# manuelinfosec/corrosion

Measured on AMD Instinct MI355X. Metric: merged column-changes/sec (node) at 1/2/4/8 GPUs + % of HBM BW roofline, higher is better.
Workload: dtype int64; 1 GPU; config 2: 64M column-changes, 1 table x 4 INTEGER cols, 1000 actors, uniform pk in [1,2^22], cl=1, one apply into an empty state per step; changes=67108864, cells=16469597, parallelism=1 GPU

## Files before the change

corrosion_amd/csrc/engine.hip:

```cpp
#include <hip/hip_runtime.h>

#include <algorithm>
#include <chrono>
#include <cstdlib>
#include <cstring>
#include <mutex>
#include <numeric>

#include "internal.h"
#include "merge_kernels.h"

namespace corro {

static thread_local std::string g_last_error;

void set_error(const std::string &msg) { g_last_error = msg; }

int fail(int code, const std::string &msg) {
    g_last_error = msg;
    return code;
}

int DevBuf::ensure(size_t want) {
    if (want <= bytes && p) return CORRO_OK;
// ... 411 lines not shown
        return fail(CORRO_E_NO_DEVICE, std::string("libcorro_hip is built for gfx950, device is ") + prop.gcnArchName);
    CORRO_HIP_TRY(hipStreamCreateWithFlags(&ctx->stream, hipStreamNonBlocking));
    CORRO_HIP_TRY(hipHostMalloc((void **)&ctx->h_misc, MISC_WORDS * sizeof(uint64_t), hipHostMallocDefault));
    CORRO_HIP_TRY(hipHostGetDevicePointer((void **)&ctx->h_misc_dev, ctx->h_misc, 0));
    for (auto &e : ctx->ev) CORRO_HIP_TRY(hipEventCreate(&e));
    const size_t lds_max = 160 * 1024;
    for (const void *f : {(const void *)k_hist<8>, (const void *)k_hist<16>, (const void *)k_hist<32>,
                          (const void *)k_hist<16, true>, (const void *)k_hist<16, false, true>})
        CORRO_HIP_TRY(hipFuncSetAttribute(f, hipFuncAttributeMaxDynamicSharedMemorySize, (int)lds_max));
    for (const void *f : {(const void *)k_scatter<true, true>, (const void *)k_scatter<true, false>,
                          (const void *)k_scatter<true, false, 8>,
                          (const void *)k_scatter<false, true>, (const void *)k_scatter<false, false>})
        CORRO_HIP_TRY(hipFuncSetAttribute(f, hipFuncAttributeMaxDynamicSharedMemorySize, (int)lds_max));
    return CORRO_OK;
}

}

static int store_alloc(corro_ctx *ctx, uint64_t capacity_hint) {
    const uint32_t B = ctx->B;
    const uint64_t rows = std::max<uint64_t>(1024, capacity_hint / 16);
    uint32_t lg = 4;
    while (((uint64_t)B << lg) < 2 * rows && lg < 20 && ((uint64_t)B << (lg + 1)) <= (1ULL << 31)) lg++;
    ctx->log2S = lg;
    TRY(ctx->d_ent.ensure(((size_t)B << lg) * sizeof(RowEnt)));
    TRY(ctx->d_used.ensure(B * 4ULL));
    TRY(ctx->d_gen.ensure(B * 4ULL));
    TRY(ctx->d_heap_top.ensure(8));
    ctx->heap_cap = std::min<uint64_t>(1ULL << 31, std::max<uint64_t>(1ULL << 16, capacity_hint / 2));
    TRY(ctx->d_heap.ensure(ctx->heap_cap * sizeof(Rec)));
    return CORRO_OK;
}

static int store_clear(corro_ctx *ctx) {
    hipStream_t s = ctx->stream;
    const size_t n16 = ((size_t)ctx->B << ctx->log2S) * (sizeof(RowEnt) / 16);
    static const uint32_t grid_max = std::getenv("CORRO_CLEAR_GRID") ? (uint32_t)std::atoi(std::getenv("CORRO_CLEAR_GRID")) : CLEAR_GRID;
    static const bool nt = !std::getenv("CORRO_CLEAR_NT") || std::atoi(std::getenv("CORRO_CLEAR_NT")) != 0;
    const uint32_t grid = (uint32_t)std::min<size_t>(std::max(grid_max, 1u), (n16 + CLEAR_T - 1) / CLEAR_T);
    hipLaunchKernelGGL(nt ? k_store_clear<true> : k_store_clear<false>, dim3(std::max(grid, 1u)), dim3(CLEAR_T), 0, s,
                       row_store(ctx), ctx->B, ctx->d_touch_n.as<unsigned long long>());
    CORRO_HIP_TRY(hipGetLastError());
    ctx->touch_bound = 0;
    ctx->state_total = 0;
    ctx->state_rows = 0;
    ctx->arena_top = 0;
    ctx->vc_last_bytes = 0;
    ctx->state_epoch++;
    ctx->poisoned = false;
    return CORRO_OK;
}

namespace corro {
RowStore row_store(corro_ctx *ctx) {
    RowStore rs{};
    rs.ent = ctx->d_ent.as<RowEnt>();
    rs.used = ctx->d_used.as<uint32_t>();
    rs.gen = ctx->d_gen.as<uint32_t>();
    rs.heap = ctx->d_heap.as<Rec>();
    rs.heap_ts = ctx->track_ts ? ctx->d_heap_ts.as<uint64_t>() : nullptr;
    rs.heap_top = ctx->d_heap_top.as<unsigned long long>();
    rs.heap_cap = ctx->heap_cap;
    rs.log2S = ctx->log2S;
    rs.fill = (uint32_t)((7ULL << ctx->log2S) >> 3);
    rs.stride = ctx->d_stride.as<uint16_t>();
    return rs;
}

static constexpr uint64_t ARENA_MAX = 1ULL << 40;
int arena_reserve(corro_ctx *ctx, uint64_t add) {
    const uint64_t need = ctx->arena_top + add;
    if (need > ARENA_MAX) return fail(CORRO_E_RANGE, "value arena would exceed 2^40 bytes");
    if (need <= ctx->d_arena.bytes && ctx->d_arena.p) return CORRO_OK;
    DevBuf nb;
    TRY(nb.ensure(std::max<uint64_t>(need + (need >> 1), 1ULL << 20)));
    if (ctx->arena_top)
        CORRO_HIP_TRY(hipMemcpyAsync(nb.p, ctx->d_arena.p, ctx->arena_top, hipMemcpyDeviceToDevice, ctx->stream));
    CORRO_HIP_TRY(hipStreamSynchronize(ctx->stream));
    ctx->d_arena.release();
    ctx->d_arena = nb;
    nb.p = nullptr;
    return CORRO_OK;
}

int grow_regions(corro_ctx *ctx, uint32_t new_log2S) {
    if (new_log2S <= ctx->log2S) return CORRO_OK;
    ctx->metrics.region_growths++;
    if (new_log2S > 26 || ((uint64_t)ctx->B << new_log2S) > (1ULL << 31))
        return fail(CORRO_E_NOMEM, "row store regions would exceed 2^31 entries");
    hipStream_t s = ctx->stream;
    DevBuf nb;
    TRY(nb.ensure(((size_t)ctx->B << new_log2S) * sizeof(RowEnt)));
    CORRO_HIP_TRY(hipMemsetAsync(nb.p, 0, ((size_t)ctx->B << new_log2S) * sizeof(RowEnt), s));
    const uint32_t old_log2S = ctx->log2S;
    DevBuf old = ctx->d_ent;
    ctx->d_ent = nb;
    nb.p = nullptr;
// ... 1090 lines not shown
```

corrosion_amd/csrc/internal.h:

```cpp
#pragma once
#include <hip/hip_runtime.h>

#include <array>
#include <cstdint>
#include <cstdlib>
#include <map>
#include <string>
#include <unordered_map>
#include <vector>

#include "corro_hip.h"

namespace corro {

inline bool fault_armed(const char *name) {
    const char *e = std::getenv("CORRO_FAULT");
    if (!e || !*e) return false;
    const std::string s = std::string(",") + e + ",";
    return s.find(std::string(",") + name + ",") != std::string::npos;
}

void set_error(const std::string &msg);
int fail(int code, const std::string &msg);

// ... 108 lines not shown
        if (o == 0xFFFFFFFFu) return o;
        if (t.lo[h] == lo && t.hi[h] == hi) return o;
        h = (h + 1) & t.mask;
    }
}

int prims_warm(corro_ctx *ctx);
int agent_dev_reserve(corro_ctx *ctx, uint64_t ncs);

}

struct corro_ctx {
    int device = 0;
    hipStream_t stream = nullptr;
    std::vector<corro::Table> tables;
    std::vector<corro::PkTable> pk;
    std::map<std::string, uint32_t> table_index;

    std::vector<std::array<uint8_t, 16>> sites;
    std::map<std::array<uint8_t, 16>, uint32_t> site_ordinal;
    corro::DevBuf d_site_rank;
    corro::DevBuf d_dbv;
    corro::DevBuf d_dbv_batch;
    size_t dbv_cap = 0;

    uint32_t log2B = 0;
    uint32_t B = 0;
    corro::DevBuf d_ent;
    corro::DevBuf d_used, d_gen;
    corro::DevBuf d_heap, d_heap_ts;
    corro::DevBuf d_heap_top;
    corro::DevBuf d_stride;
    uint32_t log2S = 0;
    uint64_t heap_cap = 0;
    uint32_t max_stride = 1;
    uint64_t state_total = 0;
    uint64_t state_rows = 0;
    corro_metrics metrics{};
    std::vector<uint64_t> committed;
    bool track_ts = false;
    bool track_touched = false;
    corro::DevBuf d_touch, d_touch_n, d_touch_stamp, d_touch_tmp;
    uint64_t touch_cap = 0;
    uint64_t touch_bound = 0;
    uint32_t touch_epoch = 0;
    uint64_t touch_stamp_n = 0;
    bool poisoned = false;
    uint64_t dbv_writes = 0;
    const uint32_t *pm_ap = nullptr, *pm_src = nullptr;
    const uint64_t *pm_ts = nullptr;
    uint64_t pm_n = 0;
    bool pm_slack = false;
    const void *slot_rec = nullptr;
    const uint64_t *slot_cnt = nullptr;
    uint32_t slot_cap = 0, slot_nsrc = 0;
    uint32_t *slot_over = nullptr;
    bool apply_wrote = false;
    uint64_t heap_limit = 0;
    bool state_wide = false;
    corro::DevBuf d_defer, d_relist;
    corro::DevBuf d_dense, d_dense_ts, d_dense_view;
    corro::DevBuf d_arena;
    uint64_t arena_top = 0;
    uint64_t vc_min_bytes = 0;
    uint64_t vc_last_bytes = 0;
    uint64_t dense_epoch = ~0ULL;
// ... 81 lines not shown
```

corrosion_amd/csrc/merge_kernels.h:

```cpp
#pragma once
#include "internal.h"
#include "rowhash.h"
#include "rowstore.h"

namespace corro {

#ifndef CORRO_DIAG
#define CORRO_DIAG 0
#endif
constexpr int HIST_THREADS = 512;
constexpr uint64_t CV_PACKED_LIMIT = 1ULL << 15;
constexpr uint32_t TILES_MAX = 256;
constexpr int MERGE_THREADS = 512;
#ifndef CORRO_FAST_T
#define CORRO_FAST_T 512
#endif
constexpr int FAST_T = CORRO_FAST_T;
constexpr int CAP_FAST = 3072;
constexpr int FAST_R = CAP_FAST / FAST_T;
static_assert(FAST_R * FAST_T == CAP_FAST, "FAST_T must divide CAP_FAST");
constexpr int FAST_WAVES_EU = 2 * (FAST_T / 64) / 4;
constexpr int FAST_SLOTS = 4096;
#ifndef IMPACT_LISTS
#define IMPACT_LISTS 0
// ... 1116 lines not shown
        if (i < n && row[k] == i) {
            s_heap[i] = 0x80000000u | off;
            off += strd[k];
        }
    }
    rows = wave_sum_u32(rows);
    if ((tid & 63) == 0 && rows) atomicAdd(&s_ctl[0], rows);
}

__device__ inline void fast_rows_alloc(const MergeArgs &a, uint32_t b, uint32_t used0, uint32_t *s_ctl,
                                       unsigned long long *s_hbase) {
    bool ok = used0 + s_ctl[0] <= a.rs.fill;
    unsigned long long h = 0;
    if (ok && s_ctl[1]) {
#if CORRO_DIAG & 8
        h = (unsigned long long)b * 640u;
#else
        h = rs_heap_alloc(a.rs, s_ctl[1]);
#endif
        ok = h != ~0ULL;
    }
    if (!ok) {
        push_defer(a, b, used0 + s_ctl[0] <= a.rs.fill ? DEFER_HEAP : DEFER_REGION);
        s_ctl[2] = 1;
    } else {
        a.rs.used[b] = used0 + s_ctl[0];
        *s_hbase = h;
    }
}

template <int R>
__device__ inline bool fast_rows(const MergeArgs &a, uint32_t b, uint32_t used0, uint32_t n, const uint32_t (&row)[R],
                                 uint32_t (&ent)[R], const uint64_t *s_pk, const uint32_t *s_tc, uint32_t *s_heap,
                                 uint64_t *s_bits, uint32_t *s_ctl, unsigned long long *s_hbase, bool counted) {
    const uint32_t tid = threadIdx.x;
    const uint32_t S = 1u << a.rs.log2S;
    uint32_t *s_bm = s_heap + CAP_FAST;
    const bool lds_claim = S <= 32 * RS_BM_WORDS;
    if (lds_claim)
        for (uint32_t w = tid; w < (S + 31) / 32; w += FAST_T) s_bm[w] = 0;
    uint32_t e0[R], hw[R];
#pragma unroll
    for (int k = 0; k < R; k++) {
        const uint32_t i = k * FAST_T + tid;
        ent[k] = ROW_NONE;
        e0[k] = 0;
        hw[k] = 0;
        if (i >= n || row[k] != i) continue;
        const uint64_t pk = s_pk[i];
        const uint32_t t = s_tc[i] >> 16;
        if (counted) {
            hw[k] = s_heap[i];
            s_bits[i] = 0;
            e0[k] = region_slot(pk, t, a.rs.log2S);
            ent[k] = ROW_NONE - 1;
            continue;
        }
        const uint32_t e = used0 ? rs_probe(a.rs, b, pk, t, e0[k]) : ROW_NONE;
        if (!used0) e0[k] = region_slot(pk, t, a.rs.log2S);
        if (e != ROW_NONE) {
            hw[k] = a.rs.ent[e].heap;
            s_bits[i] = a.rs.ent[e].bits[0];
            ent[k] = e;
        } else {
            hw[k] = (uint32_t)a.rs.stride[t];
            s_bits[i] = 0;
            ent[k] = ROW_NONE - 1;
// ... 14 lines not shown
                const uint32_t st = hw[k];
                hw[k] = 0x80000000u | off;
                off += st;
            }
        rows = wave_sum_u32(rows);
        if ((tid & 63) == 0 && rows) atomicAdd(&s_ctl[0], rows);
    }
    __syncthreads();
    if (!counted) {
#pragma unroll
        for (int k = 0; k < R; k++)
            if (ent[k] != ROW_NONE) s_heap[k * FAST_T + tid] = hw[k];
        if (tid == 0) fast_rows_alloc(a, b, used0, s_ctl, s_hbase);
        __syncthreads();
    }
    if (s_ctl[2]) return false;
#pragma unroll
    for (int k = 0; k < R; k++) {
        const uint32_t i = k * FAST_T + tid;
        if (ent[k] != ROW_NONE - 1) continue;
#if CORRO_DIAG & 2
        ent[k] = ROW_NONE;
        continue;
#endif
        const uint32_t t = s_tc[i] >> 16, hb = row_heap(hw[k], *s_hbase);
        if (!lds_claim) {
            ent[k] = rs_claim(a.rs, b, e0[k], s_pk[i], t, hb);
            continue;
        }
        uint32_t sl = e0[k];
        while (true) {
            const uint32_t bit = 1u << (sl & 31);
            if (!(atomicOr(&s_bm[sl >> 5], bit) & bit) &&
                (sl == e0[k] || !used0 || a.rs.ent[((size_t)b << a.rs.log2S) + sl].tag == 0))
                break;
            sl = (sl + 1) & (S - 1);
        }
        const uint32_t e = (b << a.rs.log2S) | sl;
        RowEnt &re = a.rs.ent[e];
        re.pk = s_pk[i];
        re.tag = t + 1;
        re.heap = hb;
        re.bits[1] = 0;
        ent[k] = e;
    }
    return true;
}

__device__ inline int prior_cmp_int(const MergeArgs &a, const Rec &pr, uint64_t cvb, uint64_t v0b, uint32_t rank) {
    const uint64_t pcv = (uint64_t)pr.cv ^ 0x8000000000000000ULL, pv = pr.v0 ^ 0x8000000000000000ULL;
    if (cvb != pcv) return cvb > pcv ? 1 : -1;
    if (v0b != pv) return v0b > pv ? 1 : -1;
    const uint32_t pr_rank = site_rank_of(a, pr.site);
    return rank != pr_rank ? (rank > pr_rank ? 1 : -1) : 0;
}

template <bool WIDE>
__device__ inline void fast_body(const MergeArgs &a, uint32_t b, const BucketView &v, bool packed = false) {
    __shared__ uint64_t s_pk[CAP_FAST];
    __shared__ uint64_t s_k[CAP_FAST];
    __shared__ uint32_t s_tc[CAP_FAST];
    __shared__ uint32_t s_own[FAST_SLOTS];
    __shared__ uint32_t s_ctl[4];
    __shared__ unsigned long long s_hbase, s_live;
    const uint32_t tid = threadIdx.x;
    const uint32_t n = v.nn;
    uint64_t cv[FAST_R], v0[FAST_R], v1[FAST_R], rp[FAST_R], dbv[FAST_R];
    uint32_t meta[FAST_R], cell[FAST_R], seq[FAST_R], site[FAST_R], row[FAST_R];
    bool alive[FAST_R];
    uint4 q[FAST_R][4];
#if CORRO_DIAG & 64
    unsigned long long diag_t = wall_clock64();
#define DIAG_MARK(k) do { if (tid == 0) { const unsigned long long t_ = wall_clock64(); atomicAdd(&a.misc[MISC_DIAG + (k)], t_ - diag_t); diag_t = t_; } } while (0)
#else
#define DIAG_MARK(k) do { } while (0)
// ... 110 lines not shown
#pragma unroll
        for (int k = 0; k < FAST_R; k++) {
            w[k] = 0;
            if (!alive[k]) continue;
            const uint32_t ty = WIDE ? vtype(meta[k]) : (uint32_t)CORRO_INTEGER;
            const bool tb = ty == CORRO_TEXT || ty == CORRO_BLOB;
            switch (which) {
            case 0: w[k] = cv[k]; break;
            case 1: w[k] = 5u - ty; break;
            case 2: w[k] = vkey0(ty, v0[k]); break;
            case 3: w[k] = tb ? v1[k] : 0; break;
            case 4: w[k] = tb ? vlen(meta[k]) : 0; break;
            default: w[k] = rp[k]; break;
            }
            atomicMax(reinterpret_cast<unsigned long long *>(&s_k[cell[k]]), (unsigned long long)w[k]);
        }
        __syncthreads();
        if (st == 0 && !used0 && tid == 0) fast_rows_alloc(a, b, used0, s_ctl, &s_hbase);
#pragma unroll
        for (int k = 0; k < FAST_R; k++)
            if (alive[k]) alive[k] = s_k[cell[k]] == w[k];
        __syncthreads();
        if (st + 1 < nstages) {
#pragma unroll
            for (int k = 0; k < FAST_R; k++) {
                const uint32_t i = k * FAST_T + tid;
                if (i < n && cell[k] == i) s_k[i] = 0;
            }
            __syncthreads();
        }
    }
    DIAG_MARK(2);
    uint32_t ent[FAST_R];
    if (!fast_rows<FAST_R>(a, b, used0, n, row, ent, s_pk, s_tc, s_own, s_k, s_ctl, &s_hbase, used0 == 0)) return;
    DIAG_MARK(3);
    uint32_t hb[FAST_R];
    uint32_t nlive = 0;
#pragma unroll
    for (int k = 0; k < FAST_R; k++) {
        hb[k] = 0;
        if (!alive[k]) continue;
        const uint32_t i = k * FAST_T + tid;
        const uint32_t c = s_tc[i] & 0xFFFFu;
        hb[k] = row_heap(s_own[row[k]], s_hbase) + c;
        if ((s_k[row[k]] >> c) & 1ULL) {
            const Rec pr = load_rec(a.rs.heap + hb[k]);
            int cmp;
            if (WIDE) {
                Rec x = load_rec(v.fresh + i);
                cmp = (int64_t)(cv[k] ^ 0x8000000000000000ULL) != pr.cv
                          ? ((int64_t)(cv[k] ^ 0x8000000000000000ULL) > pr.cv ? 1 : -1)
                          : value_cmp(x, pr, a.arena);
                if (cmp == 0) {
                    const uint32_t rk = (uint32_t)(rp[k] >> 32), prk = site_rank_of(a, pr.site);
                    cmp = rk != prk ? (rk > prk ? 1 : -1) : 0;
                }
            } else {
                cmp = prior_cmp_int(a, pr, cv[k], v0[k] ^ 0x8000000000000000ULL, (uint32_t)(rp[k] >> 32));
            }
            if (cmp <= 0) alive[k] = false;
        } else {
            atomicOr(reinterpret_cast<unsigned long long *>(&s_k[row[k]]), 1ULL << c);
            nlive++;
        }
    }
#pragma unroll
    for (int k = 0; k < FAST_R; k++) {
// ... 84 lines not shown
        alive[k] = i < n;
        cell[k] = 0;
        const Rec r = rec_from_wave_quads(q[k]);
        pk[k] = r.pk;
        tc[k] = r.tcid;
        s_pk[i] = r.pk;
        s_tc[i] = r.tcid;
        cv[k] = (uint64_t)r.cv ^ 0x8000000000000000ULL;
        v0[k] = r.v0;
        v1[k] = r.v1;
        meta[k] = r.meta;
        pos[k] = r.pos;
        site[k] = r.site;
        dbv[k] = (uint64_t)r.dbv;
        seq[k] = r.seq;
    }
#pragma unroll
    for (int k = 0; k < FAST_R; k++) rank[k] = a.site_rank[site[k] < a.nsites ? site[k] : 0u];
#pragma unroll
    for (int k = 0; k < FAST_R; k++) rank[k] = site[k] < a.nsites ? rank[k] : 0u;
    __syncthreads();
#pragma unroll
    for (int k = 0; k < FAST_R; k++) {
        const uint32_t i = k * FAST_T + tid;
        row[k] = 0;
        if (!alive[k]) continue;
        row[k] = row_claim(reinterpret_cast<uint32_t *>(s_v0), s_pk, s_tc, i, pk[k], tc[k] >> 16);
    }
    __syncthreads();
#pragma unroll
    for (int k = 0; k < FAST_R; k++)
        if (alive[k]) cell[k] = cell_claim(s_own, k * FAST_T + tid, row[k], tc[k]);
    __syncthreads();
    if (!fast_rows<FAST_R>(a, b, used0, n, row, ent, s_pk, s_tc, s_own, s_v0, s_ctl, &s_hbase, false)) return;
#pragma unroll
    for (int k = 0; k < FAST_R; k++) {
        hb[k] = 0;
        if (!alive[k]) continue;
        const uint32_t c = tc[k] & 0xFFFFu;
        hb[k] = row_heap(s_own[row[k]], s_hbase) + c;
        if ((s_v0[row[k]] >> c) & 1ULL) {
            const Rec pr = load_rec(a.rs.heap + hb[k]);
            const int64_t bcv = (int64_t)(cv[k] ^ 0x8000000000000000ULL);
            int cmp = bcv != pr.cv ? (bcv > pr.cv ? 1 : -1) : value_cmp_f(meta[k], v0[k], v1[k], pr.meta, pr.v0, pr.v1, a.arena);
            if (cmp == 0) {
                const uint32_t prk = site_rank_of(a, pr.site);
                cmp = rank[k] != prk ? (rank[k] > prk ? 1 : -1) : 0;
            }
            if (cmp > 0) flags |= 1u << (2 * k);
        } else {
            flags |= 3u << (2 * k);
        }
    }
    __syncthreads();
    for (uint32_t i = tid; i < FAST_SLOTS; i += FAST_T) s_own[i] = 0;
    __syncthreads();
#pragma unroll
    for (int k = 0; k < FAST_R; k++) {
        const uint32_t i = k * FAST_T + tid;
        if (!alive[k]) continue;
        s_pk[i] = cv[k];
        s_tc[i] = rank[k];
        s_v0[i] = v0[k];
        s_pos[i] = pos[k];
        s_v1[i] = v1[k];
        s_meta[i] = meta[k];
        atomicAdd(&s_own[cell[k]], 1u);
// ... 150 lines not shown
        alive[k] = i < n;
        cell[k] = 0;
        const Rec r = rec_from_wave_quads(q[k]);
        pk[k] = r.pk;
        tc[k] = r.tcid;
        s_a[i] = r.pk;
        s_b[i] = r.tcid;
        cv[k] = (uint64_t)r.cv ^ 0x8000000000000000ULL;
        v0[k] = r.v0 ^ 0x8000000000000000ULL;
        pos[k] = r.pos;
        site[k] = r.site;
        dbv[k] = (uint64_t)r.dbv;
        seq[k] = r.seq;
    }
#pragma unroll
    for (int k = 0; k < FAST_R; k++) rank[k] = a.site_rank[site[k] < a.nsites ? site[k] : 0u];
#pragma unroll
    for (int k = 0; k < FAST_R; k++) rank[k] = site[k] < a.nsites ? rank[k] : 0u;
    __syncthreads();
    DIAG_MARK2(0);
#pragma unroll
    for (int k = 0; k < FAST_R; k++) {
        const uint32_t i = k * FAST_T + tid;
        row[k] = 0;
        if (!alive[k]) continue;
        row[k] = row_claim(reinterpret_cast<uint32_t *>(s_c), s_a, s_b, i, pk[k], tc[k] >> 16);
    }
    __syncthreads();
#pragma unroll
    for (int k = 0; k < FAST_R; k++)
        if (alive[k]) cell[k] = cell_claim(s_own, k * FAST_T + tid, row[k], tc[k]);
    __syncthreads();
    DIAG_MARK2(1);
    if (!fast_rows<FAST_R>(a, b, used0, n, row, ent, s_a, s_b, s_own, s_c, s_ctl, &s_hbase, false)) return;
    DIAG_MARK2(2);
#pragma unroll
    for (int k = 0; k < FAST_R; k++) {
        hb[k] = 0;
        if (!alive[k]) continue;
        const uint32_t c = tc[k] & 0xFFFFu;
        hb[k] = row_heap(s_own[row[k]], s_hbase) + c;
        if ((s_c[row[k]] >> c) & 1ULL) {
            const Rec pr = load_rec(a.rs.heap + hb[k]);
            if (prior_cmp_int(a, pr, cv[k], v0[k], rank[k]) > 0) flags |= 1u << (2 * k);
        } else {
            flags |= 3u << (2 * k);
        }
    }
    __syncthreads();
    DIAG_MARK2(3);
    for (uint32_t i = tid; i < FAST_SLOTS; i += FAST_T) s_own[i] = 0;
    __syncthreads();
#pragma unroll
    for (int k = 0; k < FAST_R; k++)
        if (alive[k]) atomicAdd(&s_own[cell[k]], 1u);
    __syncthreads();
    {
        const uint32_t i0 = tid * FAST_R;
        uint32_t c[FAST_R], loc = 0;
#pragma unroll
        for (int k = 0; k < FAST_R; k++) {
            c[k] = i0 + k < n ? s_own[i0 + k] : 0u;
            loc += c[k];
        }
        const uint32_t lane = tid & 63, w = tid >> 6;
        uint32_t inc = loc;
#pragma unroll
// ... 167 lines not shown
        strd[k] = used0 ? 0u : (uint32_t)a.rs.stride[alive[k] ? tc[k] >> 16 : 0u];
        k2[k] |= a.site_rank[site[k] < a.nsites ? site[k] : 0u];
    }
#pragma unroll
    for (int k = 0; k < FAST_R; k++)
        if (site[k] >= a.nsites) k2[k] &= 0xFFFF0000u;
    __syncthreads();
    DIAG_MARK2(0);
#pragma unroll
    for (int k = 0; k < FAST_R; k++) {
        const uint32_t i = k * FAST_T + tid;
        row[k] = 0;
        if (!alive[k]) continue;
        row[k] = row_claim(reinterpret_cast<uint32_t *>(s_c), s_a, s_b, i, s_a[i], tc[k] >> 16);
    }
    __syncthreads();
#pragma unroll
    for (int k = 0; k < FAST_R; k++)
        if (alive[k]) cell[k] = cell_claim(s_own, k * FAST_T + tid, row[k], tc[k]);
    __syncthreads();
    DIAG_MARK2(1);
    unsigned long long hraw = 0;
    if (!used0) {
        fast_rows_count<FAST_R>(n, row, strd, s_own, s_ctl);
        __syncthreads();
#pragma unroll
        for (int k = 0; k < FAST_R; k++) {
            hb[k] = alive[k] ? (s_own[row[k]] & 0x7FFFFFFFu) + (tc[k] & 0xFFFFu) : 0u;
            ent[k] = ROW_NONE;
            if (alive[k]) flags |= 3u << (2 * k);
        }
        if (tid == 0 && s_ctl[1] && s_ctl[0] <= a.rs.fill) hraw = atomicAdd(a.rs.heap_top, (unsigned long long)s_ctl[1]);
    } else {
        if (!fast_rows<FAST_R>(a, b, used0, n, row, ent, s_a, s_b, s_own, s_c, s_ctl, &s_hbase, false)) return;
#pragma unroll
        for (int k = 0; k < FAST_R; k++) {
            hb[k] = 0;
            if (!alive[k]) continue;
            const uint32_t c = tc[k] & 0xFFFFu;
            hb[k] = row_heap(s_own[row[k]], s_hbase) + c;
            if ((s_c[row[k]] >> c) & 1ULL) {
                const Rec pr = load_rec(a.rs.heap + hb[k]);
                if (prior_cmp_packed(a, pr, k1[k], k2[k]) > 0) flags |= 1u << (2 * k);
            } else {
                flags |= 3u << (2 * k);
            }
        }
    }
    __syncthreads();
    DIAG_MARK2(2);
#if IMPACT_LISTS
    uint32_t *s_p = reinterpret_cast<uint32_t *>(s_c), *s_nx = s_p + CAP_FAST;
    for (uint32_t i = tid; i < CAP_FAST; i += FAST_T) s_own[i] = 0;
#pragma unroll
    for (int k = 0; k < FAST_R; k++)
        if (alive[k]) {
            const uint32_t i = k * FAST_T + tid;
            s_a[i] = k1[k];
            s_b[i] = k2[k];
            s_p[i] = pos[k];
        }
    __syncthreads();
#pragma unroll
    for (int k = 0; k < FAST_R; k++) {
        const uint32_t i = k * FAST_T + tid;
        if (alive[k] && cell[k] != i) s_nx[i] = atomicExch(&s_own[cell[k]], i + 1);
    }
// ... 88 lines not shown
            if (c > 0 || (c == 0 && earlier)) win = false;
        }
#if !(CORRO_DIAG & 1024)
        if (a.impact && (pos[k] & BATCH_POS) && imp) a.impact[pos[k] & 0x7FFFFFFFu] = 1;
#endif
        alive[k] = win;
    }
#endif
    DIAG_MARK2(5);
    if (!used0) {
        if (tid == 0) {
            const unsigned long long need = s_ctl[1];
            const bool room = s_ctl[0] <= a.rs.fill;
            if (!room || (need && hraw + need > a.rs.heap_cap)) {
                if (room && need) atomicSub(a.rs.heap_top, need);
                push_defer(a, b, room ? DEFER_HEAP : DEFER_REGION);
                s_ctl[2] = 1;
            } else {
                a.rs.used[b] = s_ctl[0];
                s_hbase = need ? hraw : 0;
            }
        }
        __syncthreads();
        if (s_ctl[2]) return;
#pragma unroll
        for (int k = 0; k < FAST_R; k++) {
            const uint32_t i = k * FAST_T + tid;
            if (i < n && row[k] == i) {
                s_a[i] = v.fresh[i].pk;
                s_b[i] = tc[k];
                s_own[i] = 0x80000000u | (hb[k] - (tc[k] & 0xFFFFu));
            }
        }
        if (!fast_rows<FAST_R>(a, b, 0u, n, row, ent, s_a, s_b, s_own, s_c, s_ctl, &s_hbase, true)) return;
#pragma unroll
        for (int k = 0; k < FAST_R; k++) hb[k] += (uint32_t)s_hbase;
    } else {
        __syncthreads();
#pragma unroll
        for (int k = 0; k < FAST_R; k++) {
            const uint32_t i = k * FAST_T + tid;
            if (ent[k] != ROW_NONE && row[k] == i) s_c[i] = a.rs.ent[ent[k]].bits[0];
        }
    }
    __syncthreads();
    DIAG_MARK2(6);
    uint32_t nlive = 0;
    constexpr int WH = (FAST_R + 1) / 2;
#pragma unroll
    for (int h = 0; h < FAST_R; h += WH) {
        uint2 w0[WH], w16[WH], w48[WH], w32[WH];
        const bool tsv = a.track_ts && a.ts_v1;
#pragma unroll
        for (int u = 0; u < WH && h + u < FAST_R; u++) {
            const int k = h + u;
            const uint32_t i = k * FAST_T + tid;
            const uint2 *src = reinterpret_cast<const uint2 *>(v.fresh + i);
            if (alive[k]) {
                w0[u] = src[0];
                w16[u] = src[2];
                w48[u] = src[6];
                if (tsv) w32[u] = src[4];
            }
        }
#pragma unroll
        for (int u = 0; u < WH && h + u < FAST_R; u++) {
            const int k = h + u;
// ... 224 lines not shown
        for (uint32_t k = 0; k < PLAN_PER / 4; k++)
            x[k] = reinterpret_cast<const uint4 *>(used)[min(threadIdx.x + k * TAIL_T, n4 - 1)];
#pragma unroll
        for (uint32_t k = 0; k < PLAN_PER / 4; k++)
            if (threadIdx.x + k * TAIL_T < n4) t += (unsigned long long)x[k].x + x[k].y + x[k].z + x[k].w;
    } else if (threadIdx.x < B) {
        t = used[threadIdx.x];
    }
    for (int d = 32; d >= 1; d >>= 1) t += __shfl_xor(t, d);
    if ((threadIdx.x & 63) == 0) s_w[threadIdx.x >> 6] = t;
    if (!misc[0])
        for (uint32_t i = threadIdx.x; i < nsites; i += TAIL_T)
            if (batch[i] > dbv[i]) dbv[i] = batch[i];
    __syncthreads();
    if (threadIdx.x < (uint32_t)MISC_WORDS) {
        unsigned long long v = misc[threadIdx.x];
        if (threadIdx.x == (uint32_t)MISC_ROWS) {
            v = 0;
            for (uint32_t ww = 0; ww < TAIL_T / 64; ww++) v += s_w[ww];
            misc[MISC_ROWS] = v;
        }
        out[threadIdx.x] = v;
    }
}

template <class F>
__device__ inline void for_each_state_record(const RowStore &rs, uint64_t nent, unsigned long long *count, F &&f) {
    const uint32_t lane = threadIdx.x & 63;
    const uint64_t stride = (uint64_t)gridDim.x * blockDim.x;
    for (uint64_t base = (uint64_t)blockIdx.x * blockDim.x + (threadIdx.x & ~63u); base < nent; base += stride) {
        const uint64_t e = base + lane;
        RowEnt re{};
        if (e < nent) re = rs.ent[e];
        const bool ok = re.tag != 0;
        const uint32_t cnt = ok ? row_popc(re.bits) : 0u;
        uint32_t inc = cnt;
#pragma unroll
        for (int d = 1; d < 64; d <<= 1) {
            const uint32_t y = __shfl_up(inc, d);
            if (lane >= (uint32_t)d) inc += y;
        }
        const uint32_t tot = __shfl(inc, 63);
        unsigned long long w0 = 0;
        if (lane == 63 && tot) w0 = atomicAdd(count, (unsigned long long)tot);
        w0 = __shfl(w0, 63);
        if (!cnt) continue;
        unsigned long long k = w0 + inc - cnt;
        const int64_t L = (re.bits[0] & 1ULL) ? rs.heap[re.heap].cv : 1;
        for (int w = 0; w < 2; w++)
            for (uint64_t m = re.bits[w]; m; m &= m - 1) {
                const uint32_t c = 64 * w + (uint32_t)__ffsll((unsigned long long)m) - 1;
                f(k++, re.heap + c, L);
            }
    }
}

__device__ inline void export_rec(const RowStore &rs, const corro_rows &o, unsigned long long k, uint32_t h, int64_t L) {
    const Rec r = load_rec(rs.heap + h);
    o.pk[k] = r.pk;
    o.table_cid[k] = r.tcid;
    o.col_version[k] = r.cv;
    o.db_version[k] = r.dbv;
    o.cl[k] = L;
    o.seq[k] = r.seq;
    o.site[k] = r.site;
    o.ts[k] = rs.heap_ts ? rs.heap_ts[h] : 0ULL;
    o.val0[k] = r.v0;
// ... 22 lines not shown
}

static __global__ void k_touch_rows(RowStore rs, const uint32_t *__restrict__ ent, const uint32_t *__restrict__ cnt,
                                    const uint32_t *__restrict__ incl, uint64_t m, corro_rows o) {
    for (uint64_t i = (uint64_t)blockIdx.x * blockDim.x + threadIdx.x; i < m; i += (uint64_t)gridDim.x * blockDim.x) {
        if (!cnt[i]) continue;
        const RowEnt re = rs.ent[ent[i]];
        unsigned long long k = incl[i] - cnt[i];
        const int64_t L = (re.bits[0] & 1ULL) ? rs.heap[re.heap].cv : 1;
        for (int w = 0; w < 2; w++)
            for (uint64_t b = re.bits[w]; b; b &= b - 1) {
                const uint32_t c = 64 * w + (uint32_t)__ffsll((unsigned long long)b) - 1;
                export_rec(rs, o, k++, re.heap + c, L);
            }
    }
}

static __global__ void k_materialize(RowStore rs, uint64_t nent, unsigned long long *count, Rec *out,
                                     uint64_t *out_ts) {
    for_each_state_record(rs, nent, count, [&](unsigned long long k, uint32_t h, int64_t L) {
        Rec r = load_rec(rs.heap + h);
        r.cl = (uint32_t)L;
        r.pos = (uint32_t)k;
        store_rec(out + k, r);
        if (out_ts) out_ts[k] = rs.heap_ts ? rs.heap_ts[h] : 0ULL;
    });
}

static __global__ void k_rehash(const RowEnt *__restrict__ old_ent, uint32_t old_log2S, RowStore rs) {
    const uint32_t b = blockIdx.x;
    const uint32_t S = 1u << old_log2S;
    for (uint32_t s = threadIdx.x; s < S; s += blockDim.x) {
        const RowEnt re = old_ent[((size_t)b << old_log2S) + s];
        if (re.tag == 0) continue;
        rs_insert(rs, b, re.pk, re.tag - 1, re.heap, re.bits);
    }
}

constexpr uint32_t CLEAR_T = 256, CLEAR_GRID = 256;
template <bool NT>
static __global__ void __launch_bounds__(CLEAR_T)
k_store_clear(RowStore rs, uint32_t B, unsigned long long *touch_n) {
    const uint32_t t = blockIdx.x * CLEAR_T + threadIdx.x, nt = gridDim.x * CLEAR_T;
    uint4 *ent = reinterpret_cast<uint4 *>(rs.ent);
    const size_t n16 = ((size_t)B << rs.log2S) * (sizeof(RowEnt) / 16);
    const uint4 zero = make_uint4(0u, 0u, 0u, 0u);
#pragma unroll 4
    for (size_t i = t; i < n16; i += nt) {
        if (NT) {
            typedef uint32_t v4u __attribute__((ext_vector_type(4)));
            const v4u z = {0u, 0u, 0u, 0u};
            __builtin_nontemporal_store(z, reinterpret_cast<v4u *>(ent + i));
        } else {
            ent[i] = zero;
        }
    }
    for (uint32_t b = t; b < B; b += nt) {
        rs.used[b] = 0;
        rs.gen[b] = 0;
    }
    if (t == 0) {
        *rs.heap_top = 0;
        if (touch_n) *touch_n = 0;
    }
}

}

// ... 2 lines not shown
```

corrosion_amd/csrc/rowstore.h:

```cpp
#pragma once
#include <hip/hip_runtime.h>

#include <cstdint>

#include "internal.h"
#include "rowhash.h"

namespace corro {

struct __attribute__((aligned(16))) RowEnt {
    uint64_t pk;
    uint32_t tag;
    uint32_t heap;
    uint64_t bits[2];
};
static_assert(sizeof(RowEnt) == 32, "RowEnt must be 32 bytes");
constexpr uint32_t ROW_NONE = 0xFFFFFFFFu;
constexpr uint32_t MAX_COLS = 127;

struct RowStore {
    RowEnt *ent;
    uint32_t *used;
    uint32_t *gen;
    Rec *heap;
    uint64_t *heap_ts;
    unsigned long long *heap_top;
    unsigned long long heap_cap;
    uint32_t log2S;
    uint32_t fill;
    const uint16_t *stride;
};

__host__ __device__ inline uint32_t region_slot(uint64_t pk, uint32_t table, uint32_t log2S) {
    const uint64_t h = mix64(pk * 0xA0761D6478BD642FULL + table + 0x51);
    return (uint32_t)(h >> 40) & ((1u << log2S) - 1u);
}

__device__ inline uint32_t row_popc(const uint64_t bits[2]) { return __popcll(bits[0]) + __popcll(bits[1]); }

__device__ inline uint32_t rs_lookup(const RowStore &rs, uint32_t b, uint64_t pk, uint32_t table) {
    const uint32_t S = 1u << rs.log2S, m = S - 1;
    const RowEnt *reg = rs.ent + ((size_t)b << rs.log2S);
    uint32_t s = region_slot(pk, table, rs.log2S);
    for (uint32_t k = 0; k < S; k++, s = (s + 1) & m) {
        const uint32_t tag = reg[s].tag;
        if (tag == 0) return ROW_NONE;
        if (tag == table + 1 && reg[s].pk == pk) return (b << rs.log2S) | s;
    }
    return ROW_NONE;
}

__device__ inline uint32_t rs_probe(const RowStore &rs, uint32_t b, uint64_t pk, uint32_t table, uint32_t &empty) {
    const uint32_t S = 1u << rs.log2S, m = S - 1;
    const RowEnt *reg = rs.ent + ((size_t)b << rs.log2S);
    uint32_t s = region_slot(pk, table, rs.log2S);
    for (uint32_t k = 0; k < S; k++, s = (s + 1) & m) {
        const uint32_t tag = reg[s].tag;
        if (tag == 0) {
            empty = s;
            return ROW_NONE;
        }
        if (tag == table + 1 && reg[s].pk == pk) return (b << rs.log2S) | s;
    }
    empty = region_slot(pk, table, rs.log2S);
    return ROW_NONE;
}

__device__ inline uint32_t rs_claim(const RowStore &rs, uint32_t b, uint32_t s, uint64_t pk, uint32_t table,
                                    uint32_t heap) {
    const uint32_t m = (1u << rs.log2S) - 1;
    RowEnt *reg = rs.ent + ((size_t)b << rs.log2S);
    while (atomicCAS(&reg[s].tag, 0u, table + 1) != 0u) s = (s + 1) & m;
    reg[s].pk = pk;
    reg[s].heap = heap;
    reg[s].bits[0] = 0;
    reg[s].bits[1] = 0;
    return (b << rs.log2S) | s;
}

__device__ inline uint32_t rs_insert(const RowStore &rs, uint32_t b, uint64_t pk, uint32_t table, uint32_t heap,
                                     const uint64_t bits[2]) {
    const uint32_t m = (1u << rs.log2S) - 1;
    RowEnt *reg = rs.ent + ((size_t)b << rs.log2S);
    uint32_t s = region_slot(pk, table, rs.log2S);
    while (true) {
        if (__hip_atomic_load(&reg[s].tag, __ATOMIC_RELAXED, __HIP_MEMORY_SCOPE_AGENT) == 0 &&
            atomicCAS(&reg[s].tag, 0u, table + 1) == 0u)
            break;
        s = (s + 1) & m;
    }
    reg[s].pk = pk;
    reg[s].heap = heap;
    reg[s].bits[0] = bits[0];
    reg[s].bits[1] = bits[1];
    return (b << rs.log2S) | s;
}

__device__ inline unsigned long long rs_heap_alloc(const RowStore &rs, unsigned long long need) {
    const unsigned long long old = atomicAdd(rs.heap_top, need);
    if (old + need <= rs.heap_cap) return old;
    atomicSub(rs.heap_top, need);
    return ~0ULL;
}

}
```

corrosion_amd/csrc/values_compact.hip:

```cpp
#include <hip/hip_runtime.h>

#include <algorithm>

#include "internal.h"
#include "merge_kernels.h"

namespace corro {

int ovf_sort_pairs(void *temp, size_t *temp_bytes, const uint64_t *ki, uint64_t *ko, const uint32_t *vi,
                   uint32_t *vo, uint32_t n, uint32_t end_bit, hipStream_t s);
int prim_inclusive_max_u64(void *temp, size_t *temp_bytes, const uint64_t *in, uint64_t *out, uint64_t n, hipStream_t s);
int prim_inclusive_sum_u64(void *temp, size_t *temp_bytes, const uint64_t *in, uint64_t *out, uint64_t n, hipStream_t s);
int prim_inclusive_scan_u32_u64(void *temp, size_t *temp_bytes, const uint32_t *in, uint64_t *out, uint64_t n,
                                hipStream_t s);
RowStore row_store(corro_ctx *ctx);

constexpr uint32_t VC_CHUNK = 4096;
constexpr uint32_t VC_GROUP = 8;

struct VcDev {
    uint64_t *off;
    uint32_t *heap;
    uint32_t *len;
    uint64_t *end;
    uint64_t *emax;
    uint64_t *gap;
    uint64_t *dead;
    uint32_t *cnt;
    uint64_t *cinc;
    uint32_t n;
};

__device__ inline bool vc_long_value(uint32_t meta) {
    const uint32_t t = vtype(meta);
    return is_long(meta) && (t == CORRO_TEXT || t == CORRO_BLOB);
}

static __global__ void k_vc_collect(RowStore rs, uint64_t nent, unsigned long long *count, uint64_t cap,
                                    uint64_t *__restrict__ off, uint32_t *__restrict__ heap) {
    const uint32_t lane = threadIdx.x & 63;
    const uint64_t stride = (uint64_t)gridDim.x * blockDim.x;
    for (uint64_t base = (uint64_t)blockIdx.x * blockDim.x + (threadIdx.x & ~63u); base < nent; base += stride) {
        const uint64_t e = base + lane;
        RowEnt re{};
        if (e < nent) re = rs.ent[e];
        uint64_t live[2] = {0, 0};
        if (re.tag != 0)
            for (int w = 0; w < 2; w++)
                for (uint64_t m = re.bits[w]; m; m &= m - 1) {
                    const uint32_t b = (uint32_t)__ffsll((unsigned long long)m) - 1;
                    if (vc_long_value(rs.heap[re.heap + 64 * w + b].meta)) live[w] |= 1ULL << b;
                }
        const uint32_t cnt = row_popc(live);
        uint32_t inc = cnt;
#pragma unroll
        for (int d = 1; d < 64; d <<= 1) {
            const uint32_t y = __shfl_up(inc, d);
            if (lane >= (uint32_t)d) inc += y;
        }
        const uint32_t tot = __shfl(inc, 63);
        unsigned long long w0 = 0;
        if (lane == 63 && tot) w0 = atomicAdd(count, (unsigned long long)tot);
        w0 = __shfl(w0, 63);
        if (!cnt || !off) continue;
        unsigned long long k = w0 + inc - cnt;
        for (int w = 0; w < 2; w++)
            for (uint64_t m = live[w]; m; m &= m - 1, k++) {
                const uint32_t h = re.heap + 64 * w + (uint32_t)__ffsll((unsigned long long)m) - 1;
                if (k >= cap) continue;
                off[k] = rs.heap[h].v1 >> 24;
                heap[k] = h;
            }
    }
}

static __global__ void k_vc_spans(VcDev d, const Rec *__restrict__ heap, uint64_t arena_top, uint32_t *__restrict__ bad) {
    for (uint32_t i = blockIdx.x * blockDim.x + threadIdx.x; i < d.n; i += gridDim.x * blockDim.x) {
        const uint64_t v1 = heap[d.heap[i]].v1, o = d.off[i], l = v1 & 0xFFFFFFu;
        if ((v1 >> 24) != o || o + l > arena_top) *bad = 1u;
        d.len[i] = (uint32_t)l;
// ... 240 lines not shown
```

Before: 18.30 billion merged column-changes/s.

## Replace full row-store clear with epoch-tagged lazy reset

Row-entry tags now carry a reset epoch in their high bits, so clearing the store just bumps the epoch and resets per-bucket used/gen counters and heap top, instead of rewriting the whole entry table. Stale entries from older epochs are treated as empty by lookup, probe, claim, collect and rehash paths. A full clear still runs when the epoch wraps. This removes a large memset-like pass per step, at the cost of slightly more complex tag checks and needing to zero bits[0] on reuse.

```diff
diff --git a/corrosion_amd/csrc/engine.hip b/corrosion_amd/csrc/engine.hip
--- a/corrosion_amd/csrc/engine.hip
+++ b/corrosion_amd/csrc/engine.hip
@@ -467,8 +467,30 @@
     return CORRO_OK;
 }
 
+static void store_cleared(corro_ctx *ctx) {
+    ctx->touch_bound = 0;
+    ctx->state_total = 0;
+    ctx->state_rows = 0;
+    ctx->arena_top = 0;
+    ctx->vc_last_bytes = 0;
+    ctx->state_epoch++;
+    ctx->poisoned = false;
+}
+
 static int store_clear(corro_ctx *ctx) {
     hipStream_t s = ctx->stream;
+    uint32_t epoch_max = EPOCH_MAX;
+    if (const char *e = std::getenv("CORRO_RESET_EPOCH_MAX"))
+        epoch_max = (uint32_t)std::min<long>(std::max<long>(std::atol(e), 1), (long)EPOCH_MAX);
+    if (ctx->reset_epoch != 0 && ctx->reset_epoch < epoch_max) {
+        ctx->reset_epoch++;
+        hipLaunchKernelGGL(k_store_reset, dim3((ctx->B + RESET_T - 1) / RESET_T), dim3(RESET_T), 0, s, row_store(ctx),
+                           ctx->B, ctx->d_touch_n.as<unsigned long long>());
+        CORRO_HIP_TRY(hipGetLastError());
+        store_cleared(ctx);
+        return CORRO_OK;
+    }
+    ctx->reset_epoch = 1;
     const size_t n16 = ((size_t)ctx->B << ctx->log2S) * (sizeof(RowEnt) / 16);
     static const uint32_t grid_max = std::getenv("CORRO_CLEAR_GRID") ? (uint32_t)std::atoi(std::getenv("CORRO_CLEAR_GRID")) : CLEAR_GRID;
     static const bool nt = !std::getenv("CORRO_CLEAR_NT") || std::atoi(std::getenv("CORRO_CLEAR_NT")) != 0;
@@ -476,13 +498,7 @@
     hipLaunchKernelGGL(nt ? k_store_clear<true> : k_store_clear<false>, dim3(std::max(grid, 1u)), dim3(CLEAR_T), 0, s,
                        row_store(ctx), ctx->B, ctx->d_touch_n.as<unsigned long long>());
     CORRO_HIP_TRY(hipGetLastError());
-    ctx->touch_bound = 0;
-    ctx->state_total = 0;
-    ctx->state_rows = 0;
-    ctx->arena_top = 0;
-    ctx->vc_last_bytes = 0;
-    ctx->state_epoch++;
-    ctx->poisoned = false;
+    store_cleared(ctx);
     return CORRO_OK;
 }
 
@@ -498,6 +514,7 @@
     rs.heap_cap = ctx->heap_cap;
     rs.log2S = ctx->log2S;
     rs.fill = (uint32_t)((7ULL << ctx->log2S) >> 3);
+    rs.etag = ctx->reset_epoch << EPOCH_SHIFT;
     rs.stride = ctx->d_stride.as<uint16_t>();
     return rs;
 }
diff --git a/corrosion_amd/csrc/internal.h b/corrosion_amd/csrc/internal.h
--- a/corrosion_amd/csrc/internal.h
+++ b/corrosion_amd/csrc/internal.h
@@ -164,6 +164,7 @@
     corro::DevBuf d_heap_top;
     corro::DevBuf d_stride;
     uint32_t log2S = 0;
+    uint32_t reset_epoch = 0;
     uint64_t heap_cap = 0;
     uint32_t max_stride = 1;
     uint64_t state_total = 0;
diff --git a/corrosion_amd/csrc/merge_kernels.h b/corrosion_amd/csrc/merge_kernels.h
--- a/corrosion_amd/csrc/merge_kernels.h
+++ b/corrosion_amd/csrc/merge_kernels.h
@@ -1172,7 +1172,8 @@
 template <int R>
 __device__ inline bool fast_rows(const MergeArgs &a, uint32_t b, uint32_t used0, uint32_t n, const uint32_t (&row)[R],
                                  uint32_t (&ent)[R], const uint64_t *s_pk, const uint32_t *s_tc, uint32_t *s_heap,
-                                 uint64_t *s_bits, uint32_t *s_ctl, unsigned long long *s_hbase, bool counted) {
+                                 uint64_t *s_bits, uint32_t *s_ctl, unsigned long long *s_hbase, bool counted,
+                                 bool zero_bits) {
     const uint32_t tid = threadIdx.x;
     const uint32_t S = 1u << a.rs.log2S;
     uint32_t *s_bm = s_heap + CAP_FAST;
@@ -1253,15 +1254,16 @@
         while (true) {
             const uint32_t bit = 1u << (sl & 31);
             if (!(atomicOr(&s_bm[sl >> 5], bit) & bit) &&
-                (sl == e0[k] || !used0 || a.rs.ent[((size_t)b << a.rs.log2S) + sl].tag == 0))
+                (sl == e0[k] || !used0 || !rs_live(a.rs, a.rs.ent[((size_t)b << a.rs.log2S) + sl].tag)))
                 break;
             sl = (sl + 1) & (S - 1);
         }
         const uint32_t e = (b << a.rs.log2S) | sl;
         RowEnt &re = a.rs.ent[e];
         re.pk = s_pk[i];
-        re.tag = t + 1;
+        re.tag = rs_tag(a.rs, t);
         re.heap = hb;
+        if (zero_bits) re.bits[0] = 0;
         re.bits[1] = 0;
         ent[k] = e;
     }
@@ -1438,7 +1440,7 @@
     }
     DIAG_MARK(2);
     uint32_t ent[FAST_R];
-    if (!fast_rows<FAST_R>(a, b, used0, n, row, ent, s_pk, s_tc, s_own, s_k, s_ctl, &s_hbase, used0 == 0)) return;
+    if (!fast_rows<FAST_R>(a, b, used0, n, row, ent, s_pk, s_tc, s_own, s_k, s_ctl, &s_hbase, used0 == 0, false)) return;
     DIAG_MARK(3);
     uint32_t hb[FAST_R];
     uint32_t nlive = 0;
@@ -1589,7 +1591,7 @@
     for (int k = 0; k < FAST_R; k++)
         if (alive[k]) cell[k] = cell_claim(s_own, k * FAST_T + tid, row[k], tc[k]);
     __syncthreads();
-    if (!fast_rows<FAST_R>(a, b, used0, n, row, ent, s_pk, s_tc, s_own, s_v0, s_ctl, &s_hbase, false)) return;
+    if (!fast_rows<FAST_R>(a, b, used0, n, row, ent, s_pk, s_tc, s_own, s_v0, s_ctl, &s_hbase, false, true)) return;
 #pragma unroll
     for (int k = 0; k < FAST_R; k++) {
         hb[k] = 0;
@@ -1806,7 +1808,7 @@
         if (alive[k]) cell[k] = cell_claim(s_own, k * FAST_T + tid, row[k], tc[k]);
     __syncthreads();
     DIAG_MARK2(1);
-    if (!fast_rows<FAST_R>(a, b, used0, n, row, ent, s_a, s_b, s_own, s_c, s_ctl, &s_hbase, false)) return;
+    if (!fast_rows<FAST_R>(a, b, used0, n, row, ent, s_a, s_b, s_own, s_c, s_ctl, &s_hbase, false, true)) return;
     DIAG_MARK2(2);
 #pragma unroll
     for (int k = 0; k < FAST_R; k++) {
@@ -2040,7 +2042,7 @@
         }
         if (tid == 0 && s_ctl[1] && s_ctl[0] <= a.rs.fill) hraw = atomicAdd(a.rs.heap_top, (unsigned long long)s_ctl[1]);
     } else {
-        if (!fast_rows<FAST_R>(a, b, used0, n, row, ent, s_a, s_b, s_own, s_c, s_ctl, &s_hbase, false)) return;
+        if (!fast_rows<FAST_R>(a, b, used0, n, row, ent, s_a, s_b, s_own, s_c, s_ctl, &s_hbase, false, true)) return;
 #pragma unroll
         for (int k = 0; k < FAST_R; k++) {
             hb[k] = 0;
@@ -2195,7 +2197,7 @@
                 s_own[i] = 0x80000000u | (hb[k] - (tc[k] & 0xFFFFu));
             }
         }
-        if (!fast_rows<FAST_R>(a, b, 0u, n, row, ent, s_a, s_b, s_own, s_c, s_ctl, &s_hbase, true)) return;
+        if (!fast_rows<FAST_R>(a, b, 0u, n, row, ent, s_a, s_b, s_own, s_c, s_ctl, &s_hbase, true, true)) return;
 #pragma unroll
         for (int k = 0; k < FAST_R; k++) hb[k] += (uint32_t)s_hbase;
     } else {
@@ -2486,7 +2488,7 @@
         const uint64_t e = base + lane;
         RowEnt re{};
         if (e < nent) re = rs.ent[e];
-        const bool ok = re.tag != 0;
+        const bool ok = rs_live(rs, re.tag);
         const uint32_t cnt = ok ? row_popc(re.bits) : 0u;
         uint32_t inc = cnt;
 #pragma unroll
@@ -2575,8 +2577,22 @@
     const uint32_t S = 1u << old_log2S;
     for (uint32_t s = threadIdx.x; s < S; s += blockDim.x) {
         const RowEnt re = old_ent[((size_t)b << old_log2S) + s];
-        if (re.tag == 0) continue;
-        rs_insert(rs, b, re.pk, re.tag - 1, re.heap, re.bits);
+        if (!rs_live(rs, re.tag)) continue;
+        rs_insert(rs, b, re.pk, tag_table(re.tag), re.heap, re.bits);
+    }
+}
+
+constexpr uint32_t RESET_T = 256;
+static __global__ void __launch_bounds__(RESET_T)
+k_store_reset(RowStore rs, uint32_t B, unsigned long long *touch_n) {
+    const uint32_t t = blockIdx.x * RESET_T + threadIdx.x;
+    if (t < B) {
+        rs.used[t] = 0;
+        rs.gen[t] = 0;
+    }
+    if (t == 0) {
+        *rs.heap_top = 0;
+        if (touch_n) *touch_n = 0;
     }
 }
 
diff --git a/corrosion_amd/csrc/rowstore.h b/corrosion_amd/csrc/rowstore.h
--- a/corrosion_amd/csrc/rowstore.h
+++ b/corrosion_amd/csrc/rowstore.h
@@ -17,6 +17,7 @@
 static_assert(sizeof(RowEnt) == 32, "RowEnt must be 32 bytes");
 constexpr uint32_t ROW_NONE = 0xFFFFFFFFu;
 constexpr uint32_t MAX_COLS = 127;
+constexpr uint32_t EPOCH_SHIFT = 16, EPOCH_MAX = 0xFFFFu;
 
 struct RowStore {
     RowEnt *ent;
@@ -28,6 +29,7 @@
     unsigned long long heap_cap;
     uint32_t log2S;
     uint32_t fill;
+    uint32_t etag;
     const uint16_t *stride;
 };
 
@@ -36,41 +38,50 @@
     return (uint32_t)(h >> 40) & ((1u << log2S) - 1u);
 }
 
+__host__ __device__ inline bool rs_live(const RowStore &rs, uint32_t tag) { return (tag >> EPOCH_SHIFT << EPOCH_SHIFT) == rs.etag; }
+__host__ __device__ inline uint32_t rs_tag(const RowStore &rs, uint32_t table) { return rs.etag | (table + 1); }
+__host__ __device__ inline uint32_t tag_table(uint32_t tag) { return (tag & ((1u << EPOCH_SHIFT) - 1u)) - 1u; }
+
 __device__ inline uint32_t row_popc(const uint64_t bits[2]) { return __popcll(bits[0]) + __popcll(bits[1]); }
 
 __device__ inline uint32_t rs_lookup(const RowStore &rs, uint32_t b, uint64_t pk, uint32_t table) {
-    const uint32_t S = 1u << rs.log2S, m = S - 1;
+    const uint32_t S = 1u << rs.log2S, m = S - 1, want = rs_tag(rs, table);
     const RowEnt *reg = rs.ent + ((size_t)b << rs.log2S);
     uint32_t s = region_slot(pk, table, rs.log2S);
     for (uint32_t k = 0; k < S; k++, s = (s + 1) & m) {
         const uint32_t tag = reg[s].tag;
-        if (tag == 0) return ROW_NONE;
-        if (tag == table + 1 && reg[s].pk == pk) return (b << rs.log2S) | s;
+        if (!rs_live(rs, tag)) return ROW_NONE;
+        if (tag == want && reg[s].pk == pk) return (b << rs.log2S) | s;
     }
     return ROW_NONE;
 }
 
 __device__ inline uint32_t rs_probe(const RowStore &rs, uint32_t b, uint64_t pk, uint32_t table, uint32_t &empty) {
-    const uint32_t S = 1u << rs.log2S, m = S - 1;
+    const uint32_t S = 1u << rs.log2S, m = S - 1, want = rs_tag(rs, table);
     const RowEnt *reg = rs.ent + ((size_t)b << rs.log2S);
     uint32_t s = region_slot(pk, table, rs.log2S);
     for (uint32_t k = 0; k < S; k++, s = (s + 1) & m) {
         const uint32_t tag = reg[s].tag;
-        if (tag == 0) {
+        if (!rs_live(rs, tag)) {
             empty = s;
             return ROW_NONE;
         }
-        if (tag == table + 1 && reg[s].pk == pk) return (b << rs.log2S) | s;
+        if (tag == want && reg[s].pk == pk) return (b << rs.log2S) | s;
     }
     empty = region_slot(pk, table, rs.log2S);
     return ROW_NONE;
+}
+
+__device__ inline bool rs_take(const RowStore &rs, uint32_t *tag, uint32_t table) {
+    const uint32_t old = __hip_atomic_load(tag, __ATOMIC_RELAXED, __HIP_MEMORY_SCOPE_AGENT);
+    return !rs_live(rs, old) && atomicCAS(tag, old, rs_tag(rs, table)) == old;
 }
 
 __device__ inline uint32_t rs_claim(const RowStore &rs, uint32_t b, uint32_t s, uint64_t pk, uint32_t table,
                                     uint32_t heap) {
     const uint32_t m = (1u << rs.log2S) - 1;
     RowEnt *reg = rs.ent + ((size_t)b << rs.log2S);
-    while (atomicCAS(&reg[s].tag, 0u, table + 1) != 0u) s = (s + 1) & m;
+    while (!rs_take(rs, &reg[s].tag, table)) s = (s + 1) & m;
     reg[s].pk = pk;
     reg[s].heap = heap;
     reg[s].bits[0] = 0;
@@ -83,12 +94,7 @@
     const uint32_t m = (1u << rs.log2S) - 1;
     RowEnt *reg = rs.ent + ((size_t)b << rs.log2S);
     uint32_t s = region_slot(pk, table, rs.log2S);
-    while (true) {
-        if (__hip_atomic_load(&reg[s].tag, __ATOMIC_RELAXED, __HIP_MEMORY_SCOPE_AGENT) == 0 &&
-            atomicCAS(&reg[s].tag, 0u, table + 1) == 0u)
-            break;
-        s = (s + 1) & m;
-    }
+    while (!rs_take(rs, &reg[s].tag, table)) s = (s + 1) & m;
     reg[s].pk = pk;
     reg[s].heap = heap;
     reg[s].bits[0] = bits[0];
diff --git a/corrosion_amd/csrc/values_compact.hip b/corrosion_amd/csrc/values_compact.hip
--- a/corrosion_amd/csrc/values_compact.hip
+++ b/corrosion_amd/csrc/values_compact.hip
@@ -45,7 +45,7 @@
         RowEnt re{};
         if (e < nent) re = rs.ent[e];
         uint64_t live[2] = {0, 0};
-        if (re.tag != 0)
+        if (rs_live(rs, re.tag))
             for (int w = 0; w < 2; w++)
                 for (uint64_t m = re.bits[w]; m; m &= m - 1) {
                     const uint32_t b = (uint32_t)__ffsll((unsigned long long)m) - 1;
```

Measured after the change: 18.44 billion merged column-changes/s, median of 6. Within noise of the previous version (+0.8%).
